# czbiohub-sf/shrimPy

Measured on AMD Instinct MI355X. Metric: voxels/sec deskew+20-iter RL deconv, 2048×2048×512 f32; HBM GB/s vs peak, higher is better.
Workload: dtype f32

## Files before the change

### shrimpy_amd/csrc/deskew.hip

```cpp

#include "resample.hpp"

#include <cstdlib>
#include <type_traits>

namespace {

constexpr int kTileY = 64;
constexpr int kTileX = 64;
constexpr int kSlabRows = 68;
constexpr int kPitch = kTileY + 1;
constexpr int kThreads = 256;
constexpr int kRowsPerThread = kTileY * kTileX / kThreads;
constexpr int kMaxAvg = 4096;

struct DeskewArgs {
  const void* in;
  float* out;
  int64_t Z, Y, X;
  int64_t Zo, Yo, Xo, Zd;
  int64_t out_pitch, out_plane;
  double a, b, c;
  int64_t oy, ox;
  int sy, sx;
  int avg_n;
  int grid;
  int tile_x;
  int64_t tiles_x, tiles_y;
  int64_t blocks;
  int xcd_swizzle;
  const float* flat_pattern;
  const float* flat_mean;
  const float* cval;
};

template <bool FLAT, bool U16 = false>
__global__ __launch_bounds__(kThreads) void deskew_kernel(DeskewArgs p) {
  using raw_t = std::conditional_t<U16, unsigned short, float>;
  __shared__ float slab[kSlabRows * kPitch];
  __shared__ float zero_row[kPitch];
  const float cv = p.cval ? p.cval[0] : 0.0f;
  if (threadIdx.x < kPitch) zero_row[threadIdx.x] = cv;

  const int tid = threadIdx.x;
  int64_t bid = blockIdx.x;
  if (p.xcd_swizzle) {
    const int64_t per = (p.blocks + 7) >> 3;
    bid = (bid & 7) * per + (bid >> 3);
    if (bid >= p.blocks) return;
  }
  const int64_t tx = bid % p.tiles_x;
  bid /= p.tiles_x;
  const int64_t ty = bid % p.tiles_y;
  const int64_t zo = bid / p.tiles_y;

  const int64_t xo0 = tx * p.tile_x;
  const int64_t yo0 = ty * kTileY;
  const int n_xo = static_cast<int>(min(static_cast<int64_t>(p.tile_x), p.Xo - xo0));
  const int n_yo = static_cast<int>(min(static_cast<int64_t>(kTileY), p.Yo - yo0));

  const int li = tid & 63;
  const int lj0 = tid >> 6;
  const double xo_d = static_cast<double>(xo0 + li);

  float acc[kRowsPerThread];
#pragma unroll
  for (int m = 0; m < kRowsPerThread; ++m) acc[m] = 0.0f;

  for (int k = 0; k < p.avg_n; ++k) {
    const int64_t zd = min(zo * p.avg_n + k, p.Zd - 1);
    const int64_t y_in = p.sy * zd + p.oy;
    const bool row_ok = (y_in >= 0) && (y_in < p.Y);

    const double zd_d = static_cast<double>(zd);
    const double z_first =
        lsr::affine_coord(zd_d, 0.0, static_cast<double>(xo0), p.a, 0.0, p.b, p.c);
    const double z_last =
        lsr::affine_coord(zd_d, 0.0, static_cast<double>(xo0 + n_xo - 1), p.a, 0.0, p.b, p.c);
    const double z_lo_d = floor(fmin(z_first, z_last));
    const double z_hi_d = floor(fmax(z_first, z_last)) + 1.0;
    const double zmax_d = static_cast<double>(p.Z - 1);
    const bool any_z = (z_hi_d >= 0.0) && (z_lo_d <= zmax_d);
    const int64_t z_lo = static_cast<int64_t>(fmin(fmax(z_lo_d, 0.0), zmax_d));
    const int64_t z_hi = static_cast<int64_t>(fmin(fmax(z_hi_d, 0.0), zmax_d));
    const int n_rows = any_z ? static_cast<int>(z_hi - z_lo + 1) : 0;

    if (k > 0) __syncthreads();
    if (row_ok && n_rows > 0) {
      const int col = tid & 63;
      const int j = (p.sx > 0) ? col : (kTileY - 1 - col);
      const int64_t x_in = p.sx * (yo0 + j) + p.ox;
      const bool col_ok = (j < n_yo) && (x_in >= 0) && (x_in < p.X);
      const int64_t x_safe = min(max(x_in, static_cast<int64_t>(0)), p.X - 1);
      const raw_t* src = static_cast<const raw_t*>(p.in) + (z_lo * p.Y + y_in) * p.X + x_safe;
      const int64_t z_stride = p.Y * p.X;
      float pat = 1.0f, mean = 1.0f;
      if constexpr (FLAT) {
        pat = p.flat_pattern[y_in * p.X + x_safe];
        mean = p.flat_mean[0];
      }
      constexpr int kStep = kThreads / 64;
      constexpr int kBatch = 6;
      for (int zl0 = tid >> 6; zl0 < n_rows; zl0 += kStep * kBatch) {
        float v[kBatch];
#pragma unroll
        for (int i = 0; i < kBatch; ++i) v[i] = static_cast<float>(src[min(zl0 + i * kStep, n_rows - 1) * z_stride]);
#pragma unroll
        for (int i = 0; i < kBatch; ++i) {
          const int zl = zl0 + i * kStep;
          if (zl < n_rows) {
            float w = v[i];
            if constexpr (FLAT) w = w / pat * mean;
            slab[zl * kPitch + j] = col_ok ? w : cv;
          }
        }
      }
    }
    __syncthreads();

    const double z_in = lsr::affine_coord(zd_d, 0.0, xo_d, p.a, 0.0, p.b, p.c);
    const bool ok = row_ok && (li < n_xo) &&
                    (p.grid ? (z_in > -1.0 && z_in < zmax_d + 1.0) : (!(z_in < 0.0) && !(z_in > zmax_d)));
    if (ok) {
      const double zf = floor(z_in);
      double w0, w1;
      lsr::tap_weights(z_in - zf, w0, w1);
      const int64_t z0 = static_cast<int64_t>(zf);
      const int r0 = static_cast<int>(max(z0, static_cast<int64_t>(0)) - z_lo);
      const int r1 = static_cast<int>(min(z0 + 1, p.Z - 1) - z_lo);
      const float* s0 = z0 < 0 ? zero_row : slab + r0 * kPitch;
      const float* s1 = (p.grid && z0 + 1 > p.Z - 1) ? zero_row : slab + r1 * kPitch;
#pragma unroll
      for (int m = 0; m < kRowsPerThread; ++m) {
        const int j = lj0 + 4 * m;
        double t = lsr::dadd(0.0, lsr::dmul(static_cast<double>(s0[j]), w0));
        t = lsr::dadd(t, lsr::dmul(static_cast<double>(s1[j]), w1));
        const float d = static_cast<float>(t);
        acc[m] = (k == 0) ? d : (acc[m] + d);
      }
    } else {
#pragma unroll
      for (int m = 0; m < kRowsPerThread; ++m) acc[m] = (k == 0) ? cv : (acc[m] + cv);
    }
  }

  if (li < n_xo) {
    const float denom = static_cast<float>(p.avg_n);
    float* dst = p.out + zo * p.out_plane + yo0 * p.out_pitch + xo0 + li;
#pragma unroll
    for (int m = 0; m < kRowsPerThread; ++m) {
      const int j = lj0 + 4 * m;
      if (j < n_yo) dst[static_cast<int64_t>(j) * p.out_pitch] = (p.avg_n > 1) ? acc[m] / denom : acc[m];
    }
  }
}

__global__ __launch_bounds__(256) void average_slices_kernel(const float* __restrict__ in,
                                                             float* __restrict__ out, int64_t Zd,
                                                             int64_t plane, int64_t Zo,
                                                             int avg_n) {
  const int64_t total = Zo * plane;
  const int64_t stride = static_cast<int64_t>(gridDim.x) * blockDim.x;
  for (int64_t i = static_cast<int64_t>(blockIdx.x) * blockDim.x + threadIdx.x; i < total;
       i += stride) {
    const int64_t zo = i / plane;
    const int64_t r = i - zo * plane;
    float acc = 0.0f;
    for (int k = 0; k < avg_n; ++k) {
      const int64_t zd = min(zo * avg_n + k, Zd - 1);
      const float d = in[zd * plane + r];
      acc = (k == 0) ? d : (acc + d);
    }
    out[i] = (avg_n > 1) ? acc / static_cast<float>(avg_n) : acc;
  }
}

bool is_integer(double v) { return v == static_cast<double>(static_cast<int64_t>(v)); }

}

namespace {

int deskew_impl(const char* what, const void* in, bool u16, int64_t Z, int64_t Y, int64_t X, float* out,
                int64_t Zo, int64_t Yo, int64_t Xo, int64_t out_pitch, int64_t out_plane,
                int64_t Zd, const double M[12], int avg_n, const float* flat_pattern,
                const float* flat_mean, lsr_stream_t stream, int mode = LSR_MODE_CONSTANT, const float* cval = nullptr) {
  LSR_REQUIRE_PTR(in);
  LSR_REQUIRE(mode == LSR_MODE_CONSTANT || mode == LSR_MODE_GRID_CONSTANT, LSR_E_ARG,
              "mode %d: LSR_MODE_CONSTANT or LSR_MODE_GRID_CONSTANT", mode);
  LSR_REQUIRE_PTR(out);
  LSR_REQUIRE_PTR(M);
  LSR_REQUIRE(Z > 0 && Y > 0 && X > 0, LSR_E_SHAPE, "raw shape (%lld,%lld,%lld) must be positive",
              (long long)Z, (long long)Y, (long long)X);
  LSR_REQUIRE_VOLUME(Z, Y, X);
  LSR_REQUIRE(Zo > 0 && Yo > 0 && Xo > 0 && Zd > 0, LSR_E_SHAPE,
              "output shape (%lld,%lld,%lld) / Zd %lld must be positive", (long long)Zo,
              (long long)Yo, (long long)Xo, (long long)Zd);
  LSR_REQUIRE_VOLUME(Zo, Yo, Xo);
  LSR_REQUIRE_VOLUME(Zd, Yo, Xo);
  LSR_REQUIRE(avg_n >= 1 && avg_n <= kMaxAvg, LSR_E_ARG, "avg_n %d outside [1,%d]", avg_n,
              kMaxAvg);
  LSR_REQUIRE(Zo == lsr::ceil_div(Zd, avg_n), LSR_E_SHAPE,
              "Zo %lld != ceil(Zd %lld / avg_n %d)", (long long)Zo, (long long)Zd, avg_n);
  LSR_REQUIRE_STRIDES(out_pitch, out_plane);
  LSR_REQUIRE(out_pitch >= Xo && out_plane >= Yo * out_pitch, LSR_E_SHAPE,
              "output strides (%lld, %lld) are smaller than the output plane (%lld x %lld)",
              (long long)out_pitch, (long long)out_plane, (long long)Yo, (long long)Xo);
  if (int rc = lsr::check_matrix(M)) return rc;

  const bool structured = M[1] == 0.0 && (M[4] == 1.0 || M[4] == -1.0) && M[5] == 0.0 &&
                          M[6] == 0.0 && is_integer(M[7]) && M[8] == 0.0 &&
                          (M[9] == 1.0 || M[9] == -1.0) && M[10] == 0.0 && is_integer(M[11]);
  LSR_REQUIRE(structured, LSR_E_UNSUPPORTED,
              "matrix is not a deskew shear (rows 1,2 must be signed unit axes with integer "
              "offsets, M[0][1] == 0): use lsr_affine_f32 + lsr_average_slices_f32");

  DeskewArgs p;
  p.in = in;
  p.out = out;
  p.Z = Z; p.Y = Y; p.X = X;
  p.Zo = Zo; p.Yo = Yo; p.Xo = Xo; p.Zd = Zd;
  p.out_pitch = out_pitch; p.out_plane = out_plane;
  p.a = M[0]; p.b = M[2]; p.c = M[3];
  p.sy = static_cast<int>(M[4]); p.oy = static_cast<int64_t>(M[7]);
  p.sx = static_cast<int>(M[9]); p.ox = static_cast<int64_t>(M[11]);
  p.avg_n = avg_n;
  p.grid = mode == LSR_MODE_GRID_CONSTANT ? 1 : 0;

  const double ab = p.b < 0 ? -p.b : p.b;
  int tile_x = kTileX;
  while (tile_x > 1 && ab * (tile_x - 1) + 3.0 > static_cast<double>(kSlabRows)) tile_x >>= 1;
  LSR_REQUIRE(ab * (tile_x - 1) + 3.0 <= static_cast<double>(kSlabRows), LSR_E_UNSUPPORTED,
              "scan step per output voxel |b| = %g is too large for the LDS slab", ab);
  p.tile_x = tile_x;
  p.tiles_x = lsr::ceil_div(Xo, tile_x);
  p.tiles_y = lsr::ceil_div(Yo, kTileY);
  const int64_t blocks = p.tiles_x * p.tiles_y * Zo;
  LSR_REQUIRE(blocks < (int64_t(1) << 31), LSR_E_SHAPE, "grid of %lld workgroups is too large",
              (long long)blocks);

  p.flat_pattern = flat_pattern;
  p.flat_mean = flat_mean;
  p.cval = cval;
  p.blocks = blocks;
  p.xcd_swizzle = 1;
  if (const char* e = std::getenv("LSR_DESKEW_SWIZZLE")) p.xcd_swizzle = e[0] != '0';
  const dim3 grid(static_cast<unsigned>(p.xcd_swizzle ? 8 * ((blocks + 7) / 8) : blocks)), block(kThreads);
  hipStream_t s = lsr::as_stream(stream);
  if (u16 && flat_pattern != nullptr) hipLaunchKernelGGL((deskew_kernel<true, true>), grid, block, 0, s, p);
  else if (u16) hipLaunchKernelGGL((deskew_kernel<false, true>), grid, block, 0, s, p);
  else if (flat_pattern != nullptr) hipLaunchKernelGGL((deskew_kernel<true, false>), grid, block, 0, s, p);
  else hipLaunchKernelGGL((deskew_kernel<false, false>), grid, block, 0, s, p);
  return lsr::launch_status(what);
}

}

extern "C" int lsr_deskew_f32(const float* in, int64_t Z, int64_t Y, int64_t X, float* out,
                              int64_t Zo, int64_t Yo, int64_t Xo, int64_t out_pitch,
                              int64_t out_plane, int64_t Zd, const double M[12], int avg_n,
                              lsr_stream_t stream) {
  return deskew_impl("lsr_deskew_f32", in, false, Z, Y, X, out, Zo, Yo, Xo, out_pitch, out_plane, Zd, M,
                     avg_n, nullptr, nullptr, stream);
}

extern "C" int lsr_deskew_u16(const uint16_t* in, int64_t Z, int64_t Y, int64_t X, float* out,
                              int64_t Zo, int64_t Yo, int64_t Xo, int64_t out_pitch,
                              int64_t out_plane, int64_t Zd, const double M[12], int avg_n,
                              lsr_stream_t stream) {
  return deskew_impl("lsr_deskew_u16", in, true, Z, Y, X, out, Zo, Yo, Xo, out_pitch, out_plane, Zd, M,
                     avg_n, nullptr, nullptr, stream);
}

extern "C" int lsr_deskew_flat_u16(const uint16_t* in, int64_t Z, int64_t Y, int64_t X, float* out,
                                   int64_t Zo, int64_t Yo, int64_t Xo, int64_t out_pitch,
                                   int64_t out_plane, int64_t Zd, const double M[12], int avg_n,
                                   const float* flat_pattern, const float* flat_mean,
                                   lsr_stream_t stream) {
  LSR_REQUIRE_PTR(flat_pattern);
  LSR_REQUIRE_PTR(flat_mean);
  return deskew_impl("lsr_deskew_flat_u16", in, true, Z, Y, X, out, Zo, Yo, Xo, out_pitch, out_plane, Zd,
                     M, avg_n, flat_pattern, flat_mean, stream);
}

extern "C" int lsr_deskew_flat_f32(const float* in, int64_t Z, int64_t Y, int64_t X, float* out,
                                   int64_t Zo, int64_t Yo, int64_t Xo, int64_t out_pitch,
                                   int64_t out_plane, int64_t Zd, const double M[12], int avg_n,
                                   const float* flat_pattern, const float* flat_mean,
                                   lsr_stream_t stream) {
  LSR_REQUIRE_PTR(flat_pattern);
  LSR_REQUIRE_PTR(flat_mean);
  return deskew_impl("lsr_deskew_flat_f32", in, false, Z, Y, X, out, Zo, Yo, Xo, out_pitch, out_plane, Zd,
                     M, avg_n, flat_pattern, flat_mean, stream);
}

extern "C" int lsr_deskew_border(const void* in, int in_u16, int64_t Z, int64_t Y, int64_t X, float* out,
                                 int64_t Zo, int64_t Yo, int64_t Xo, int64_t out_pitch, int64_t out_plane,
                                 int64_t Zd, const double M[12], int avg_n, int mode, const float* flat_pattern,
                                 const float* flat_mean, lsr_stream_t stream) {
  LSR_REQUIRE((flat_pattern == nullptr) == (flat_mean == nullptr), LSR_E_NULL,
              "flat_pattern and flat_mean come together (both NULL: no flat-field correction)");
  return deskew_impl("lsr_deskew_border", in, in_u16 != 0, Z, Y, X, out, Zo, Yo, Xo, out_pitch, out_plane, Zd, M,
                     avg_n, flat_pattern, flat_mean, stream, mode);
}

extern "C" int lsr_deskew_cval(const void* in, int in_u16, int64_t Z, int64_t Y, int64_t X, float* out,
                               int64_t Zo, int64_t Yo, int64_t Xo, int64_t out_pitch, int64_t out_plane,
                               int64_t Zd, const double M[12], int avg_n, int mode, const float* flat_pattern,
                               const float* flat_mean, const float* cval, lsr_stream_t stream) {
  LSR_REQUIRE((flat_pattern == nullptr) == (flat_mean == nullptr), LSR_E_NULL,
              "flat_pattern and flat_mean come together (both NULL: no flat-field correction)");
  return deskew_impl("lsr_deskew_cval", in, in_u16 != 0, Z, Y, X, out, Zo, Yo, Xo, out_pitch, out_plane, Zd, M,
                     avg_n, flat_pattern, flat_mean, stream, mode, cval);
}

extern "C" int lsr_average_slices_f32(const float* in, int64_t Zd, int64_t Y, int64_t X,
                                      float* out, int64_t Zo, int avg_n, lsr_stream_t stream) {
  LSR_REQUIRE_PTR(in);
  LSR_REQUIRE_PTR(out);
  LSR_REQUIRE(Zd > 0 && Y > 0 && X > 0 && Zo > 0, LSR_E_SHAPE, "shape must be positive");
  LSR_REQUIRE_VOLUME(Zd, Y, X);
  LSR_REQUIRE_VOLUME(Zo, Y, X);
  LSR_REQUIRE(avg_n >= 1 && avg_n <= kMaxAvg, LSR_E_ARG, "avg_n %d outside [1,%d]", avg_n,
              kMaxAvg);
  LSR_REQUIRE(Zo == lsr::ceil_div(Zd, avg_n), LSR_E_SHAPE, "Zo %lld != ceil(Zd %lld / avg_n %d)",
              (long long)Zo, (long long)Zd, avg_n);
  const int64_t plane = Y * X;
  const int64_t total = Zo * plane;
  const int64_t blocks = lsr::ceil_div(total, 256) < 8192 ? lsr::ceil_div(total, 256) : 8192;
  hipLaunchKernelGGL(average_slices_kernel, dim3(static_cast<unsigned>(blocks)), dim3(256), 0,
                     lsr::as_stream(stream), in, out, Zd, plane, Zo, avg_n);
  return lsr::launch_status("lsr_average_slices_f32");
}
```

Measured before the change: 40.17 billion.

## Use buffer loads/stores, 32-bit indexing, and non-temporal stores in deskew kernel

Rewrites the deskew kernel to use AMD buffer resource loads and stores with per-row bounds, narrowing most index arithmetic to 32-bit and unsigned block decoding. Slab fill becomes branchless using a column mask, wave index and slab bounds go to scalar registers via readfirstlane, and the first averaging plane is specialized. Output stores can use a non-temporal hint when alignment allows. The aim is fewer VALU address instructions and less cache pollution from the streaming output. The risk is 32-bit overflow on large volumes and relying on buffer out-of-range semantics for masking.

Result: no change. 40.51 billion, median of 6 (+0.9%).

```diff
diff --git a/shrimpy_amd/csrc/deskew.hip b/shrimpy_amd/csrc/deskew.hip
--- a/shrimpy_amd/csrc/deskew.hip
+++ b/shrimpy_amd/csrc/deskew.hip
@@ -17,8 +17,8 @@
 struct DeskewArgs {
   const void* in;
   float* out;
-  int64_t Z, Y, X;
-  int64_t Zo, Yo, Xo, Zd;
+  int Z, Y, X;
+  int Yo, Xo, Zd;
   int64_t out_pitch, out_plane;
   double a, b, c;
   int64_t oy, ox;
@@ -26,50 +26,80 @@
   int avg_n;
   int grid;
   int tile_x;
-  int64_t tiles_x, tiles_y;
-  int64_t blocks;
+  unsigned tiles_x, tiles_y;
+  unsigned blocks;
   int xcd_swizzle;
+  int nt_stores;
   const float* flat_pattern;
   const float* flat_mean;
   const float* cval;
 };
 
+using rsrc_t = __amdgpu_buffer_rsrc_t;
+template <typename T>
+__device__ __forceinline__ rsrc_t row_rsrc(const T* row, unsigned bytes) {
+  return __builtin_amdgcn_make_buffer_rsrc(const_cast<T*>(row), 0, static_cast<int>(bytes), 0x00020000);
+}
+__device__ __forceinline__ float row_load(rsrc_t row, unsigned byte_off, float) {
+  return __uint_as_float(__builtin_amdgcn_raw_buffer_load_b32(row, byte_off, 0, 0));
+}
+__device__ __forceinline__ float row_load(rsrc_t row, unsigned byte_off, unsigned short) {
+  return static_cast<float>(__builtin_amdgcn_raw_buffer_load_b16(row, byte_off, 0, 0));
+}
+template <bool NT>
+__device__ __forceinline__ void row_store(rsrc_t row, unsigned byte_off, float v) {
+  __builtin_amdgcn_raw_buffer_store_b32(__float_as_uint(v), row, byte_off, 0, NT ? 2 : 0);
+}
+
 template <bool FLAT, bool U16 = false>
 __global__ __launch_bounds__(kThreads) void deskew_kernel(DeskewArgs p) {
   using raw_t = std::conditional_t<U16, unsigned short, float>;
-  __shared__ float slab[kSlabRows * kPitch];
-  __shared__ float zero_row[kPitch];
+  __shared__ float lds[(kSlabRows + 1) * kPitch];
+  constexpr int kZeroRow = kSlabRows * kPitch;
   const float cv = p.cval ? p.cval[0] : 0.0f;
-  if (threadIdx.x < kPitch) zero_row[threadIdx.x] = cv;
-
   const int tid = threadIdx.x;
-  int64_t bid = blockIdx.x;
+  if (tid < kPitch) lds[kZeroRow + tid] = cv;
+
+  unsigned bid = blockIdx.x;
   if (p.xcd_swizzle) {
-    const int64_t per = (p.blocks + 7) >> 3;
+    const unsigned per = (p.blocks + 7) >> 3;
     bid = (bid & 7) * per + (bid >> 3);
     if (bid >= p.blocks) return;
   }
-  const int64_t tx = bid % p.tiles_x;
+  const unsigned tx = bid % p.tiles_x;
   bid /= p.tiles_x;
-  const int64_t ty = bid % p.tiles_y;
-  const int64_t zo = bid / p.tiles_y;
-
-  const int64_t xo0 = tx * p.tile_x;
-  const int64_t yo0 = ty * kTileY;
-  const int n_xo = static_cast<int>(min(static_cast<int64_t>(p.tile_x), p.Xo - xo0));
-  const int n_yo = static_cast<int>(min(static_cast<int64_t>(kTileY), p.Yo - yo0));
+  const unsigned ty = bid % p.tiles_y;
+  const int zo = static_cast<int>(bid / p.tiles_y);
+
+  const int xo0 = static_cast<int>(tx) * p.tile_x;
+  const int yo0 = static_cast<int>(ty) * kTileY;
+  const int n_xo = min(p.tile_x, p.Xo - xo0);
+  const int n_yo = min(kTileY, p.Yo - yo0);
 
   const int li = tid & 63;
-  const int lj0 = tid >> 6;
+  const int wave = __builtin_amdgcn_readfirstlane(tid >> 6);
   const double xo_d = static_cast<double>(xo0 + li);
+  const double zmax_d = static_cast<double>(p.Z - 1);
+
+  const int j_st = (p.sx > 0) ? li : (kTileY - 1 - li);
+  const int64_t x_in = p.sx * static_cast<int64_t>(yo0 + j_st) + p.ox;
+  const bool col_ok = (j_st < n_yo) && (x_in >= 0) && (x_in < p.X);
+  unsigned col_mask = col_ok ? ~0u : 0u;
+  asm("" : "+v"(col_mask));
+  const unsigned cv_bits = __float_as_uint(cv) & ~col_mask;
+  const unsigned x_safe = static_cast<unsigned>(min(max(x_in, static_cast<int64_t>(0)), static_cast<int64_t>(p.X - 1)));
+  const unsigned src_off = x_safe * static_cast<unsigned>(sizeof(raw_t));
+  const unsigned row_bytes = static_cast<unsigned>(p.X) * static_cast<unsigned>(sizeof(raw_t));
+  const int64_t z_stride = static_cast<int64_t>(p.Y) * p.X;
+  float mean = 1.0f;
+  if constexpr (FLAT) mean = p.flat_mean[0];
 
   float acc[kRowsPerThread];
-#pragma unroll
-  for (int m = 0; m < kRowsPerThread; ++m) acc[m] = 0.0f;
-
-  for (int k = 0; k < p.avg_n; ++k) {
-    const int64_t zd = min(zo * p.avg_n + k, p.Zd - 1);
-    const int64_t y_in = p.sy * zd + p.oy;
+
+  auto plane = [&](const int k, auto first) {
+    constexpr bool FIRST = decltype(first)::value;
+    const int zd = min(zo * p.avg_n + k, p.Zd - 1);
+    const int64_t y_in = p.sy * static_cast<int64_t>(zd) + p.oy;
     const bool row_ok = (y_in >= 0) && (y_in < p.Y);
 
     const double zd_d = static_cast<double>(zd);
@@ -79,78 +109,76 @@
         lsr::affine_coord(zd_d, 0.0, static_cast<double>(xo0 + n_xo - 1), p.a, 0.0, p.b, p.c);
     const double z_lo_d = floor(fmin(z_first, z_last));
     const double z_hi_d = floor(fmax(z_first, z_last)) + 1.0;
-    const double zmax_d = static_cast<double>(p.Z - 1);
     const bool any_z = (z_hi_d >= 0.0) && (z_lo_d <= zmax_d);
-    const int64_t z_lo = static_cast<int64_t>(fmin(fmax(z_lo_d, 0.0), zmax_d));
-    const int64_t z_hi = static_cast<int64_t>(fmin(fmax(z_hi_d, 0.0), zmax_d));
-    const int n_rows = any_z ? static_cast<int>(z_hi - z_lo + 1) : 0;
-
-    if (k > 0) __syncthreads();
+    const int z_lo = __builtin_amdgcn_readfirstlane(static_cast<int>(fmin(fmax(z_lo_d, 0.0), zmax_d)));
+    const int z_hi = __builtin_amdgcn_readfirstlane(static_cast<int>(fmin(fmax(z_hi_d, 0.0), zmax_d)));
+    const int n_rows = __builtin_amdgcn_readfirstlane(any_z ? z_hi - z_lo + 1 : 0);
+
+    if (!FIRST) __syncthreads();
     if (row_ok && n_rows > 0) {
-      const int col = tid & 63;
-      const int j = (p.sx > 0) ? col : (kTileY - 1 - col);
-      const int64_t x_in = p.sx * (yo0 + j) + p.ox;
-      const bool col_ok = (j < n_yo) && (x_in >= 0) && (x_in < p.X);
-      const int64_t x_safe = min(max(x_in, static_cast<int64_t>(0)), p.X - 1);
-      const raw_t* src = static_cast<const raw_t*>(p.in) + (z_lo * p.Y + y_in) * p.X + x_safe;
-      const int64_t z_stride = p.Y * p.X;
-      float pat = 1.0f, mean = 1.0f;
-      if constexpr (FLAT) {
-        pat = p.flat_pattern[y_in * p.X + x_safe];
-        mean = p.flat_mean[0];
-      }
+      const raw_t* src = static_cast<const raw_t*>(p.in) + (static_cast<int64_t>(z_lo) * p.Y + y_in) * p.X;
+      float pat = 1.0f;
+      if constexpr (FLAT) pat = row_load(row_rsrc(p.flat_pattern + y_in * p.X, static_cast<unsigned>(p.X) * 4u), x_safe * 4u, float());
       constexpr int kStep = kThreads / 64;
       constexpr int kBatch = 6;
-      for (int zl0 = tid >> 6; zl0 < n_rows; zl0 += kStep * kBatch) {
+      for (int zl0 = wave; zl0 < n_rows; zl0 += kStep * kBatch) {
         float v[kBatch];
 #pragma unroll
-        for (int i = 0; i < kBatch; ++i) v[i] = static_cast<float>(src[min(zl0 + i * kStep, n_rows - 1) * z_stride]);
+        for (int i = 0; i < kBatch; ++i)
+          v[i] = row_load(row_rsrc(src + static_cast<unsigned>(min(zl0 + i * kStep, n_rows - 1)) * z_stride, row_bytes), src_off, raw_t());
 #pragma unroll
         for (int i = 0; i < kBatch; ++i) {
-          const int zl = zl0 + i * kStep;
-          if (zl < n_rows) {
-            float w = v[i];
-            if constexpr (FLAT) w = w / pat * mean;
-            slab[zl * kPitch + j] = col_ok ? w : cv;
-          }
+          float w = v[i];
+          if constexpr (FLAT) w = w / pat * mean;
+          lds[min(zl0 + i * kStep, n_rows - 1) * kPitch + j_st] = __uint_as_float((__float_as_uint(w) & col_mask) | cv_bits);
         }
       }
     }
     __syncthreads();
 
     const double z_in = lsr::affine_coord(zd_d, 0.0, xo_d, p.a, 0.0, p.b, p.c);
-    const bool ok = row_ok && (li < n_xo) &&
-                    (p.grid ? (z_in > -1.0 && z_in < zmax_d + 1.0) : (!(z_in < 0.0) && !(z_in > zmax_d)));
+    const bool in_z = p.grid ? ((z_in > -1.0) & (z_in < zmax_d + 1.0)) : (!(z_in < 0.0) & !(z_in > zmax_d));
+    const bool ok = row_ok & (li < n_xo) & in_z;
     if (ok) {
       const double zf = floor(z_in);
       double w0, w1;
       lsr::tap_weights(z_in - zf, w0, w1);
-      const int64_t z0 = static_cast<int64_t>(zf);
-      const int r0 = static_cast<int>(max(z0, static_cast<int64_t>(0)) - z_lo);
-      const int r1 = static_cast<int>(min(z0 + 1, p.Z - 1) - z_lo);
-      const float* s0 = z0 < 0 ? zero_row : slab + r0 * kPitch;
-      const float* s1 = (p.grid && z0 + 1 > p.Z - 1) ? zero_row : slab + r1 * kPitch;
+      const int z0 = static_cast<int>(zf);
+      const int o0 = z0 < 0 ? kZeroRow : (max(z0, 0) - z_lo) * kPitch;
+      const int o1 = (p.grid && z0 + 1 > p.Z - 1) ? kZeroRow : (min(z0 + 1, p.Z - 1) - z_lo) * kPitch;
+      const float* s0 = lds + o0 + wave;
+      const float* s1 = lds + o1 + wave;
 #pragma unroll
       for (int m = 0; m < kRowsPerThread; ++m) {
-        const int j = lj0 + 4 * m;
-        double t = lsr::dadd(0.0, lsr::dmul(static_cast<double>(s0[j]), w0));
-        t = lsr::dadd(t, lsr::dmul(static_cast<double>(s1[j]), w1));
+        double t = lsr::dadd(0.0, lsr::dmul(static_cast<double>(s0[4 * m]), w0));
+        t = lsr::dadd(t, lsr::dmul(static_cast<double>(s1[4 * m]), w1));
         const float d = static_cast<float>(t);
-        acc[m] = (k == 0) ? d : (acc[m] + d);
+        acc[m] = FIRST ? d : (acc[m] + d);
       }
     } else {
 #pragma unroll
-      for (int m = 0; m < kRowsPerThread; ++m) acc[m] = (k == 0) ? cv : (acc[m] + cv);
+      for (int m = 0; m < kRowsPerThread; ++m) acc[m] = FIRST ? cv : (acc[m] + cv);
     }
+  };
+  plane(0, std::true_type{});
+  for (int k = 1; k < p.avg_n; ++k) plane(k, std::false_type{});
+
+  if (p.avg_n > 1) {
+    const float denom = static_cast<float>(p.avg_n);
+#pragma unroll
+    for (int m = 0; m < kRowsPerThread; ++m) acc[m] = acc[m] / denom;
   }
-
   if (li < n_xo) {
-    const float denom = static_cast<float>(p.avg_n);
-    float* dst = p.out + zo * p.out_plane + yo0 * p.out_pitch + xo0 + li;
-#pragma unroll
-    for (int m = 0; m < kRowsPerThread; ++m) {
-      const int j = lj0 + 4 * m;
-      if (j < n_yo) dst[static_cast<int64_t>(j) * p.out_pitch] = (p.avg_n > 1) ? acc[m] / denom : acc[m];
+    float* dst = p.out + zo * p.out_plane + (yo0 + wave) * p.out_pitch + xo0;
+    const unsigned dst_off = static_cast<unsigned>(li) * 4u;
+    if (p.nt_stores) {
+#pragma unroll
+      for (int m = 0; m < kRowsPerThread; ++m)
+        row_store<true>(row_rsrc(dst + (4 * m) * p.out_pitch, wave + 4 * m < n_yo ? n_xo * 4u : 0u), dst_off, acc[m]);
+    } else {
+#pragma unroll
+      for (int m = 0; m < kRowsPerThread; ++m)
+        row_store<false>(row_rsrc(dst + (4 * m) * p.out_pitch, wave + 4 * m < n_yo ? n_xo * 4u : 0u), dst_off, acc[m]);
     }
   }
 }
@@ -218,8 +246,8 @@
   DeskewArgs p;
   p.in = in;
   p.out = out;
-  p.Z = Z; p.Y = Y; p.X = X;
-  p.Zo = Zo; p.Yo = Yo; p.Xo = Xo; p.Zd = Zd;
+  p.Z = static_cast<int>(Z); p.Y = static_cast<int>(Y); p.X = static_cast<int>(X);
+  p.Yo = static_cast<int>(Yo); p.Xo = static_cast<int>(Xo); p.Zd = static_cast<int>(Zd);
   p.out_pitch = out_pitch; p.out_plane = out_plane;
   p.a = M[0]; p.b = M[2]; p.c = M[3];
   p.sy = static_cast<int>(M[4]); p.oy = static_cast<int64_t>(M[7]);
@@ -233,18 +261,21 @@
   LSR_REQUIRE(ab * (tile_x - 1) + 3.0 <= static_cast<double>(kSlabRows), LSR_E_UNSUPPORTED,
               "scan step per output voxel |b| = %g is too large for the LDS slab", ab);
   p.tile_x = tile_x;
-  p.tiles_x = lsr::ceil_div(Xo, tile_x);
-  p.tiles_y = lsr::ceil_div(Yo, kTileY);
-  const int64_t blocks = p.tiles_x * p.tiles_y * Zo;
+  const int64_t tiles_x = lsr::ceil_div(Xo, tile_x), tiles_y = lsr::ceil_div(Yo, kTileY);
+  const int64_t blocks = tiles_x * tiles_y * Zo;
   LSR_REQUIRE(blocks < (int64_t(1) << 31), LSR_E_SHAPE, "grid of %lld workgroups is too large",
               (long long)blocks);
 
   p.flat_pattern = flat_pattern;
   p.flat_mean = flat_mean;
   p.cval = cval;
-  p.blocks = blocks;
+  p.tiles_x = static_cast<unsigned>(tiles_x);
+  p.tiles_y = static_cast<unsigned>(tiles_y);
+  p.blocks = static_cast<unsigned>(blocks);
   p.xcd_swizzle = 1;
   if (const char* e = std::getenv("LSR_DESKEW_SWIZZLE")) p.xcd_swizzle = e[0] != '0';
+  p.nt_stores = tile_x == kTileX && reinterpret_cast<uintptr_t>(out) % 128 == 0 && out_pitch % 32 == 0 && out_plane % 32 == 0;
+  if (const char* e = std::getenv("LSR_DESKEW_NT")) p.nt_stores = e[0] != '0';
   const dim3 grid(static_cast<unsigned>(p.xcd_swizzle ? 8 * ((blocks + 7) / 8) : blocks)), block(kThreads);
   hipStream_t s = lsr::as_stream(stream);
   if (u16 && flat_pattern != nullptr) hipLaunchKernelGGL((deskew_kernel<true, true>), grid, block, 0, s, p);
```
